# teddyjfpender/tstwo

Measured on AMD Instinct MI355X. Metric: M31 CFFT elems/sec at log_size=22 (per step: CFFT evaluate + Blake2s Merkle commit + root all-gather), higher is better.
Workload: dtype u32

## Files before the change

tstwo_amd/csrc/common.h:

```cpp
#pragma once
#include <hip/hip_runtime.h>
#include <stdint.h>
#include <stdio.h>
#include <initializer_list>
#include <string>

#include "../../include/tstwo_hip.h"
#include "host_field.h"
#include "m31.cuh"

namespace tstwo {

struct Context {
    bool ready = false;
    int device = -1;
    hipStream_t own_stream = nullptr;
    hipStream_t stream = nullptr;
    cpoint *gen_pow2 = nullptr;
    cpoint *gen_win = nullptr;
    u32 *flag = nullptr;
    u32 *flag_host = nullptr;
    u32 *scratch = nullptr;
    size_t scratch_bytes = 0;
    int n_cus = 256;
    u32 **coltab = nullptr;
    size_t coltab_cap = 0;
    void *pinned = nullptr;
    void *result_host = nullptr;
    void *result_dev = nullptr;
    void *up_ring = nullptr;
    hipEvent_t up_done[16] = {};
    bool up_busy[16] = {};
    int up_next = 0;
    u32 *seq_host = nullptr;
    u32 *seq_dev = nullptr;
    u32 seq_next = 0;
    hipStream_t copy_stream[2] = {nullptr, nullptr};
    hipEvent_t copy_after = nullptr;
    hipEvent_t copy_done[2] = {nullptr, nullptr};
    bool copy_pending[2] = {false, false};
    int copy_next = 0;
};
constexpr size_t kPinnedBytes = 64 * 1024;
constexpr size_t kResultBytes = 256 * 1024;
constexpr int kUpSlots = 16;
constexpr int kCopyStreams = 2;
constexpr size_t kUpSlotBytes = 16 * 1024;

struct Knobs {
    int cfft_rounds = 1;
    int cfft_maxwg = 0;
    int cfft_lds_pad = 0;
    int cfft_kb = 0, cfft_ka = 0;
    int cfft_logta = 0;
    bool cfft_trace = false, cfft_sync = false;
    int merkle_cap = 32;
    int fold_cap = 64;
};
#ifdef TSTWO_EXPERIMENTS
const Knobs &knobs();
#else
inline constexpr Knobs kShippedKnobs{};
inline constexpr const Knobs &knobs() { return kShippedKnobs; }
#endif

Context &ctx();
int set_error(int code, const char *msg);
int set_error(int code, const std::string &msg);
int hip_fail(hipError_t e, const char *what);
int require_ready();
int ensure_scratch(size_t bytes);
bool stream_is_capturing();
int wait_stream();
int read_and_clear_flag(u32 *value);
int small_d2h(void *host_dst, const void *dev_src, size_t bytes);
void *result_target(size_t bytes);
int result_wait(const void **host_view);
int small_h2d(void *dev_dst, const void *host_src, size_t bytes);

#define TSTWO_HIP(call)                                        \
    do {                                                       \
        hipError_t _e = (call);                                \
        if (_e != hipSuccess) return ::tstwo::hip_fail(_e, #call); \
    } while (0)

#define TSTWO_REQUIRE_READY()                      \
    do {                                           \
        int _rc = ::tstwo::require_ready();        \
        if (_rc) return _rc;                       \
    } while (0)

#define TSTWO_LAUNCH_CHECK() TSTWO_HIP(hipGetLastError())

static inline unsigned ceil_div(size_t a, size_t b) { return (unsigned)((a + b - 1) / b); }

constexpr int kMaxColsPerLaunch = 64;
struct ColPtrs { u32 *p[kMaxColsPerLaunch]; u32 *const *ext; };
#ifdef __HIPCC__
typedef u32 u32x4_t __attribute__((ext_vector_type(4)));
typedef u32 u32x2_t __attribute__((ext_vector_type(2)));
#define TSTWO_GLOBAL __attribute__((address_space(1)))
__device__ __forceinline__ void raise_flag(u32 *flag) { *(volatile TSTWO_GLOBAL u32 *)flag = 1u; }
template <bool NT, class V>
__device__ __forceinline__ V gload_as(const TSTWO_GLOBAL V *p) {
    if constexpr (NT) return __builtin_nontemporal_load(p);
    else return *p;
}
template <bool NT, class V>
__device__ __forceinline__ void gstore_as(TSTWO_GLOBAL V *p, V v) {
    if constexpr (NT) __builtin_nontemporal_store(v, p);
    else *p = v;
}
template <bool NT = false>
__device__ __forceinline__ uint4 gload4(const u32 *p) {
    const u32x4_t v = gload_as<NT>((const TSTWO_GLOBAL u32x4_t *)p);
    return make_uint4(v.x, v.y, v.z, v.w);
}
__device__ __forceinline__ uint2 gload2(const u32 *p) {
    const u32x2_t v = *(const TSTWO_GLOBAL u32x2_t *)p;
    return make_uint2(v.x, v.y);
}
template <bool NT = false>
__device__ __forceinline__ u32 gload1(const u32 *p) { return gload_as<NT>((const TSTWO_GLOBAL u32 *)p); }
template <bool NT = false>
__device__ __forceinline__ void gstore4(u32 *p, uint4 x) {
    u32x4_t v;
    v.x = x.x; v.y = x.y; v.z = x.z; v.w = x.w;
    gstore_as<NT>((TSTWO_GLOBAL u32x4_t *)p, v);
}
template <bool NT = false>
__device__ __forceinline__ void gstore1(u32 *p, u32 x) { gstore_as<NT>((TSTWO_GLOBAL u32 *)p, x); }
template <bool NT = false>
__device__ __forceinline__ uint4 gload4(const u32 *base, u32 word_off) {
    const u32x4_t v = gload_as<NT>((const TSTWO_GLOBAL u32x4_t *)((const TSTWO_GLOBAL char *)base + (word_off << 2)));
    return make_uint4(v.x, v.y, v.z, v.w);
}
__device__ __forceinline__ uint2 gload2(const u32 *base, u32 word_off) {
    const u32x2_t v = *(const TSTWO_GLOBAL u32x2_t *)((const TSTWO_GLOBAL char *)base + (word_off << 2));
    return make_uint2(v.x, v.y);
}
template <bool NT = false>
__device__ __forceinline__ u32 gload1(const u32 *base, u32 word_off) { return gload_as<NT>((const TSTWO_GLOBAL u32 *)((const TSTWO_GLOBAL char *)base + (word_off << 2))); }
template <bool NT = false>
__device__ __forceinline__ void gstore4(u32 *base, u32 word_off, uint4 x) {
    u32x4_t v;
    v.x = x.x; v.y = x.y; v.z = x.z; v.w = x.w;
    gstore_as<NT>((TSTWO_GLOBAL u32x4_t *)((TSTWO_GLOBAL char *)base + (word_off << 2)), v);
}
__device__ __forceinline__ void gstore2(u32 *base, u32 word_off, uint2 x) {
    u32x2_t v;
    v.x = x.x; v.y = x.y;
    *(TSTWO_GLOBAL u32x2_t *)((TSTWO_GLOBAL char *)base + (word_off << 2)) = v;
}
template <bool NT = false>
__device__ __forceinline__ void gstore1(u32 *base, u32 word_off, u32 x) { gstore_as<NT>((TSTWO_GLOBAL u32 *)((TSTWO_GLOBAL char *)base + (word_off << 2)), x); }
__device__ __forceinline__ u32 *colp(const ColPtrs &c, u32 i) {
    u32 *p;
    if (c.ext) {
        asm volatile("");
        p = c.ext[i];
    } else {
        p = c.p[i];
    }
    return p;
}
template <int KERNARG_OFF = 0>
__device__ __forceinline__ u32 *colp_u(const ColPtrs &c, u32 i) {
    typedef const unsigned long long __attribute__((address_space(4))) *k64;
    typedef const char __attribute__((address_space(4))) *kbytes;
    const k64 tab = c.ext ? (k64)(unsigned long long)c.ext : (k64)((kbytes)__builtin_amdgcn_kernarg_segment_ptr() + KERNARG_OFF);
    u32 *p = (u32 *)tab[(u32)__builtin_amdgcn_readfirstlane((int)i)];
    return p;
}
constexpr int kSecondTableOff = (int)sizeof(ColPtrs);
#endif
int merkle_commit_then_channel(const u32 *const *cols, const u32 *log_sizes, size_t n_cols, uint8_t *layers, u32 *chan, u32 *felt,
                               const u32 *const *fold_in, const u32 *inv_x, const u32 *alpha_dev);
int launch_fri_tail(u32 *const (*eval)[4], uint8_t *const *trees, u32 n_layers, u32 log0, const u32 *itw, u32 tw_log, u32 *chan, u32 *alphas,
                    const u32 *const *pre, const u32 *pre_alpha);
__attribute__((visibility("hidden"))) int download_roots(const uint8_t *const *layers, size_t n_trees, uint8_t *roots);
__attribute__((visibility("hidden"))) void air_native_shutdown();
int fill_col_table(ColPtrs &out, const u32 *const *cols, size_t n_cols, int slot);
constexpr int kMaxHashCols = 256;
struct HashColPtrs { const u32 *p[kMaxHashCols]; };
struct Soa4 { u32 *p[4]; };
struct CSoa4 { const u32 *p[4]; };

inline bool has_null(std::initializer_list<const void *> l) {
    for (const void *p : l) if (!p) return true;
    return false;
}
template <typename T>
inline bool table_has_null(T *const *t, size_t n) {
    if (!t) return n > 0;
    for (size_t i = 0; i < n; i++) if (!t[i]) return true;
    return false;
}
#define TSTWO_REQUIRE_PTRS(...) do { if (::tstwo::has_null({__VA_ARGS__})) return set_error(TSTWO_ERR_BAD_ARG, "null device pointer"); } while (0)
#define TSTWO_REQUIRE_TABLE(t, n) do { if (::tstwo::table_has_null((t), (n))) return set_error(TSTWO_ERR_BAD_ARG, "null device pointer in table"); } while (0)
inline bool aligned16(const void *p) { return ((uintptr_t)p & 15) == 0; }
inline qm31 to_q(const u32 a[4]) { return {a[0], a[1], a[2], a[3]}; }
inline qm31 to_q(host::Q a) { return {a.v[0], a.v[1], a.v[2], a.v[3]}; }
inline host::Q to_hq(const u32 a[4]) { host::Q q; for (int i = 0; i < 4; i++) q.v[i] = a[i]; return q; }

}
```

tstwo_amd/csrc/context.hip:

```cpp
#include "common.h"

#include <stdlib.h>
#include <string.h>

#include <chrono>
#include <map>
#include <mutex>
#include <unordered_map>
#include <vector>

namespace tstwo {

static Context g_ctx;
static thread_local std::string g_last_error;

Context &ctx() { return g_ctx; }

#ifdef TSTWO_EXPERIMENTS
static Knobs read_knobs() {
    Knobs k;
    auto num = [](const char *name, int dflt) { const char *e = getenv(name); return e && *e ? atoi(e) : dflt; };
    auto on = [](const char *name) { return getenv(name) != nullptr; };
    k.cfft_rounds = num("TSTWO_CFFT_ROUNDS", 1); if (k.cfft_rounds < 1) k.cfft_rounds = 1;
    k.cfft_maxwg = num("TSTWO_CFFT_MAXWG", 0); if (k.cfft_maxwg < 0) k.cfft_maxwg = 0;
    k.cfft_lds_pad = num("TSTWO_CFFT_LDS_PAD", 0);
    k.cfft_kb = num("TSTWO_CFFT_KB", 0); if (k.cfft_kb < 11 || k.cfft_kb > 15) k.cfft_kb = 0;
    k.cfft_ka = num("TSTWO_CFFT_KA", 0); if (k.cfft_ka < 1 || k.cfft_ka > 10) k.cfft_ka = 0;
    k.cfft_logta = num("TSTWO_CFFT_LOGTA", 0); if (k.cfft_logta < 12 || k.cfft_logta > 15) k.cfft_logta = 0;
    k.cfft_trace = on("TSTWO_CFFT_TRACE"); k.cfft_sync = on("TSTWO_CFFT_SYNC");
    k.merkle_cap = num("TSTWO_MERKLE_CAP", 32);
    k.fold_cap = num("TSTWO_FOLD_CAP", 64);
    return k;
}
const Knobs &knobs() {
    static const Knobs k = read_knobs();
    return k;
}
#endif

int set_error(int code, const char *msg) {
    g_last_error = msg ? msg : "";
    return code;
}
int set_error(int code, const std::string &msg) {
    g_last_error = msg;
    return code;
}
int hip_fail(hipError_t e, const char *what) {
    g_last_error = std::string("HIP error: ") + hipGetErrorString(e) + " in " + what;
    (void)hipGetLastError();
    return TSTWO_ERR_HIP;
}
int require_ready() {
    if (!g_ctx.ready) {
        int rc = tstwo_init(0);
        if (rc) return rc;
    }
    return TSTWO_OK;
}
bool stream_is_capturing() {
    hipStreamCaptureStatus st = hipStreamCaptureStatusNone;
    if (hipStreamIsCapturing(g_ctx.stream, &st) != hipSuccess) { (void)hipGetLastError(); return false; }
    return st != hipStreamCaptureStatusNone;
}
static std::vector<void *> g_scratch_retired;
int ensure_scratch(size_t bytes) {
    Context &c = g_ctx;
    if (c.scratch_bytes >= bytes) return TSTWO_OK;
    size_t want = bytes < (1u << 20) ? (1u << 20) : bytes;
    if (c.scratch) {
        if (stream_is_capturing())
            return set_error(TSTWO_ERR_BAD_ARG, "scratch growth during graph capture (run the sequence once eagerly first: the "
                                                "library's scratch block must already hold what the captured calls need)");
        if (want < 2 * c.scratch_bytes) want = 2 * c.scratch_bytes;
    }
    u32 *grown = nullptr;
    TSTWO_HIP(hipMalloc((void **)&grown, want));
    if (c.scratch) g_scratch_retired.push_back(c.scratch);
    c.scratch = grown;
    c.scratch_bytes = want;
    return TSTWO_OK;
}
__global__ void k_signal(u32 *seq, u32 value) { *(volatile TSTWO_GLOBAL u32 *)seq = value; }
int wait_stream() {
    Context &c = g_ctx;
    if (!c.seq_host) {
        TSTWO_HIP(hipStreamSynchronize(c.stream));
        return TSTWO_OK;
    }
    const u32 want = ++c.seq_next;
    hipLaunchKernelGGL(k_signal, dim3(1), dim3(1), 0, c.stream, c.seq_dev, want);
    if (hipGetLastError() != hipSuccess) {
        TSTWO_HIP(hipStreamSynchronize(c.stream));
        return TSTWO_OK;
    }
    const auto t0 = std::chrono::steady_clock::now();
    for (unsigned spins = 0;; spins++) {
        if (__atomic_load_n(c.seq_host, __ATOMIC_ACQUIRE) == want) return TSTWO_OK;
        if ((spins & 255u) == 255u && std::chrono::steady_clock::now() - t0 > std::chrono::microseconds(100)) break;
    }
    TSTWO_HIP(hipStreamSynchronize(c.stream));
    return TSTWO_OK;
}
int small_d2h(void *host_dst, const void *dev_src, size_t bytes) {
    Context &c = g_ctx;
    if (bytes == 0) return TSTWO_OK;
    if (!c.pinned || bytes > kPinnedBytes) {
        TSTWO_HIP(hipMemcpyAsync(host_dst, dev_src, bytes, hipMemcpyDeviceToHost, c.stream));
        TSTWO_HIP(hipStreamSynchronize(c.stream));
        return TSTWO_OK;
    }
    TSTWO_HIP(hipMemcpyAsync(c.pinned, dev_src, bytes, hipMemcpyDeviceToHost, c.stream));
    if (int rc = wait_stream()) return rc;
    memcpy(host_dst, c.pinned, bytes);
    return TSTWO_OK;
}
void *result_target(size_t bytes) {
    Context &c = g_ctx;
    return (c.result_dev && bytes <= kResultBytes) ? c.result_dev : nullptr;
}
int result_wait(const void **host_view) {
    Context &c = g_ctx;
    if (int rc = wait_stream()) return rc;
    *host_view = c.result_host;
    return TSTWO_OK;
}
static int refuse_if_capturing() {
    if (stream_is_capturing())
        return set_error(TSTWO_ERR_BAD_ARG, "host-array upload during graph capture (column tables beyond 64 pointers, gather "
                                            "requests and quotient constants cannot be recorded)");
    return TSTWO_OK;
}
int small_h2d(void *dev_dst, const void *host_src, size_t bytes) {
    Context &c = g_ctx;
    if (bytes == 0) return TSTWO_OK;
    if (int rc = refuse_if_capturing()) return rc;
    if (!c.up_ring || bytes > kUpSlotBytes) {
        TSTWO_HIP(hipMemcpyAsync(dev_dst, host_src, bytes, hipMemcpyHostToDevice, c.stream));
        TSTWO_HIP(hipStreamSynchronize(c.stream));
        return TSTWO_OK;
    }
    const int k = c.up_next;
    c.up_next = (k + 1) % kUpSlots;
    if (c.up_busy[k]) TSTWO_HIP(hipEventSynchronize(c.up_done[k]));
    unsigned char *slot = (unsigned char *)c.up_ring + (size_t)k * kUpSlotBytes;
    memcpy(slot, host_src, bytes);
    TSTWO_HIP(hipMemcpyAsync(dev_dst, slot, bytes, hipMemcpyHostToDevice, c.stream));
    TSTWO_HIP(hipEventRecord(c.up_done[k], c.stream));
    c.up_busy[k] = true;
    return TSTWO_OK;
}
static std::vector<const u32 *> g_coltab_last[2];
static u32 **g_coltab_last_base[2] = {nullptr, nullptr};
static void coltab_cache_reset() { for (int i = 0; i < 2; i++) { g_coltab_last[i].clear(); g_coltab_last_base[i] = nullptr; } }

int fill_col_table(ColPtrs &out, const u32 *const *cols, size_t n_cols, int slot) {
    Context &c = g_ctx;
    out.ext = nullptr;
    if (n_cols <= (size_t)kMaxColsPerLaunch) {
        for (size_t i = 0; i < (size_t)kMaxColsPerLaunch; i++) out.p[i] = const_cast<u32 *>(cols[i < n_cols ? i : 0]);
        return TSTWO_OK;
    }
    if (int rc = refuse_if_capturing()) return rc;
    if (c.coltab_cap < n_cols) {
        size_t cap = 1024;
        while (cap < n_cols) cap *= 2;
        if (c.coltab) {
            TSTWO_HIP(hipStreamSynchronize(c.stream));
            TSTWO_HIP(hipFree(c.coltab));
            c.coltab = nullptr;
            c.coltab_cap = 0;
            coltab_cache_reset();
        }
        TSTWO_HIP(hipMalloc((void **)&c.coltab, 2 * cap * sizeof(u32 *)));
        c.coltab_cap = cap;
    }
    u32 **dst = c.coltab + (size_t)(slot & 1) * c.coltab_cap;
    std::vector<const u32 *> &lc = g_coltab_last[slot & 1];
    u32 ***last_base = g_coltab_last_base;
    if (!(last_base[slot & 1] == dst && lc.size() == n_cols && memcmp(lc.data(), cols, n_cols * sizeof(u32 *)) == 0)) {
        int rc = small_h2d(dst, cols, n_cols * sizeof(u32 *));
        if (rc) return rc;
        lc.assign(cols, cols + n_cols);
// ... 536 lines not shown
```

tstwo_amd/csrc/merkle.hip:

```cpp
#include <string.h>

#include <vector>

#include "blake2s.cuh"
#include "common.h"

using namespace tstwo;
using namespace tstwo::b2s;

namespace {

struct LayerParams {
    u32 total_words;
    u32 w_begin;
    u32 w_end;
    u32 col_word0;
    u32 n_cols;
    u32 load_state;
    u32 is_final;
};

template <bool HAS_PREV>
__device__ __forceinline__ void load_block(u32 (&m)[16], const uint4 *__restrict__ prev, const HashColPtrs &cols,
                                           const LayerParams &lp, size_t node, u32 w) {
    if (HAS_PREV && w == 0) {
        const uint4 *c = prev + 4 * node;
        uint4 c0 = c[0], c1 = c[1], c2 = c[2], c3 = c[3];
        m[0] = c0.x; m[1] = c0.y; m[2] = c0.z; m[3] = c0.w; m[4] = c1.x; m[5] = c1.y; m[6] = c1.z; m[7] = c1.w;
        m[8] = c2.x; m[9] = c2.y; m[10] = c2.z; m[11] = c2.w; m[12] = c3.x; m[13] = c3.y; m[14] = c3.z; m[15] = c3.w;
    } else if (lp.n_cols == 0) {
#pragma unroll
        for (int k = 0; k < 16; k++) m[k] = 0u;
    } else {
        const u32 last = lp.n_cols - 1u;
#pragma unroll
        for (int k = 0; k < 16; k++) {
            const u32 ci = w + (u32)k - lp.col_word0;
            const u32 v = cols.p[min(ci, last)][node];
            m[k] = (ci <= last) ? v : 0u;
        }
    }
}

template <bool HAS_PREV>
__global__ void __launch_bounds__(256) k_merkle_layer(const uint4 *__restrict__ prev, HashColPtrs cols, uint4 *__restrict__ out,
                                                     size_t n_nodes, LayerParams lp) {
    const size_t stride = (size_t)gridDim.x * blockDim.x;
    const size_t node0 = (size_t)blockIdx.x * blockDim.x + threadIdx.x;
    const u32 W = lp.total_words;
    const u32 w_stop = lp.w_end < W ? lp.w_end : W;
    const u32 nb = w_stop > lp.w_begin ? (w_stop - lp.w_begin + 15u) / 16u : 1u;
    const u32 rows = (u32)((n_nodes + stride - 1) / stride);
    const u32 total = rows * nb;
    const size_t last_node = n_nodes - 1;

    u32 ma[16], mb[16], h[8];
    u32 j = 0, blk = 0;
    load_block<HAS_PREV>(ma, prev, cols, lp, min(node0, last_node), lp.w_begin);

#define MERKLE_STEP(CUR, NXT)                                                                                         \
    {                                                                                                                 \
        const size_t node = node0 + (size_t)j * stride;                                                               \
        const size_t nc = min(node, last_node);                                                                       \
        const u32 wc = lp.w_begin + 16u * blk;                                                                        \
        if (blk == 0) {                                                                                               \
            if (lp.load_state) {                                                                                      \
                uint4 a = out[2 * nc], b = out[2 * nc + 1];                                                           \
                h[0] = a.x; h[1] = a.y; h[2] = a.z; h[3] = a.w; h[4] = b.x; h[5] = b.y; h[6] = b.z; h[7] = b.w;       \
            } else {                                                                                                  \
                h[0] = IV0 ^ 0x01010020u; h[1] = IV1; h[2] = IV2; h[3] = IV3; h[4] = IV4; h[5] = IV5; h[6] = IV6; h[7] = IV7; \
            }                                                                                                         \
        }                                                                                                             \
        u32 jn = j, bn = blk + 1;                                                                                     \
        if (bn == nb) { bn = 0; jn = j + 1; }                                                                         \
        if (it + 1 < total)                                                                                           \
            load_block<HAS_PREV>(NXT, prev, cols, lp, min(node0 + (size_t)jn * stride, last_node), lp.w_begin + 16u * bn); \
        const u32 bytes_end = (wc + 16 < W ? wc + 16 : W) * 4u;                                                       \
        b2s_compress(h, CUR, bytes_end, lp.is_final && (wc + 16 >= W));                                               \
        if (blk + 1 == nb && node < n_nodes) {                                                                        \
            out[2 * node] = make_uint4(h[0], h[1], h[2], h[3]);                                                       \
            out[2 * node + 1] = make_uint4(h[4], h[5], h[6], h[7]);                                                   \
        }                                                                                                             \
        j = jn; blk = bn;                                                                                             \
    }

    for (u32 it = 0; it < total; it += 2) {
        MERKLE_STEP(ma, mb)
        if (it + 1 < total) {
            const u32 it_save = it;
            it = it_save + 1;
            MERKLE_STEP(mb, ma)
            it = it_save;
        }
    }
#undef MERKLE_STEP
}

constexpr int kMaxTrees = 8;
struct TreeSet { uint4 *t[kMaxTrees]; };
template <int NBLK>
__global__ void __launch_bounds__(256) k_merkle_leaf_static(HashColPtrs cols, TreeSet outs, size_t n_nodes) {
    uint4 *__restrict__ out = outs.t[blockIdx.y];
    const u32 col0 = blockIdx.y * (16 * NBLK);
    const size_t stride = (size_t)gridDim.x * blockDim.x;
    const size_t node0 = (size_t)blockIdx.x * blockDim.x + threadIdx.x;
    const u32 rows = (u32)((n_nodes + stride - 1) / stride);
    const size_t last_node = n_nodes - 1;
    u32 cur[16], nxt[16];
    auto word = [&](int k, u32 byte_off) -> u32 { return *(const TSTWO_GLOBAL u32 *)((const TSTWO_GLOBAL char *)cols.p[col0 + k] + byte_off); };
    {
        const u32 oc = (u32)min(node0, last_node) * 4u;
#pragma unroll
        for (int k = 0; k < 16; k++) cur[k] = word(k, oc);
    }
    u32 hp[8] = {0, 0, 0, 0, 0, 0, 0, 0};
    size_t pnode = n_nodes;
    for (u32 j = 0; j < rows; j++) {
        const size_t node = node0 + (size_t)j * stride;
        const size_t nn = min(node + stride, last_node);
        const size_t nc = min(node, last_node);
        u32 h[8] = {IV0 ^ 0x01010020u, IV1, IV2, IV3, IV4, IV5, IV6, IV7};
#pragma unroll
        for (int b = 0; b < NBLK; b++) {
            const int bn = (b + 1) % NBLK;
            const u32 src = (u32)((b + 1 < NBLK) ? nc : nn) * 4u;
#pragma unroll
            for (int k = 0; k < 16; k++) nxt[k] = word(16 * bn + k, src);
            if (b == 0 && pnode < n_nodes) {
                out[2 * pnode] = make_uint4(hp[0], hp[1], hp[2], hp[3]);
                out[2 * pnode + 1] = make_uint4(hp[4], hp[5], hp[6], hp[7]);
            }
            b2s_compress(h, cur, 64u * (b + 1), b == NBLK - 1);
#pragma unroll
            for (int k = 0; k < 16; k++) cur[k] = nxt[k];
        }
#pragma unroll
        for (int k = 0; k < 8; k++) hp[k] = h[k];
        pnode = node;
    }
    if (pnode < n_nodes) {
        out[2 * pnode] = make_uint4(hp[0], hp[1], hp[2], hp[3]);
        out[2 * pnode + 1] = make_uint4(hp[4], hp[5], hp[6], hp[7]);
    }
}

struct FoldSpec { const u32 *in[4]; const u32 *inv_x; const u32 *alpha; };
struct FoldRow { uint2 a, b, c, d; u32 t; };
__device__ __forceinline__ FoldRow fold_row_load(const FoldSpec &fs, size_t i) {
    return {gload2(fs.in[0] + 2 * i), gload2(fs.in[1] + 2 * i), gload2(fs.in[2] + 2 * i), gload2(fs.in[3] + 2 * i), gload1(fs.inv_x + i)};
}
__device__ __forceinline__ qm31 fold_row(const FoldRow &r, qm31 alpha) {
    const qm31 f0 = {m31_add(r.a.x, r.a.y), m31_add(r.b.x, r.b.y), m31_add(r.c.x, r.c.y), m31_add(r.d.x, r.d.y)};
    const qm31 f1 = qm31_mul_m31({m31_sub(r.a.x, r.a.y), m31_sub(r.b.x, r.b.y), m31_sub(r.c.x, r.c.y), m31_sub(r.d.x, r.d.y)}, r.t);
    return qm31_add(f0, qm31_mul(alpha, f1));
}

template <bool FOLD>
__global__ void __launch_bounds__(256) k_merkle_leaf4(u32 *__restrict__ c0, u32 *__restrict__ c1, u32 *__restrict__ c2, u32 *__restrict__ c3,
                                                     uint4 *__restrict__ out, size_t n_nodes, FoldSpec fs) {
    const size_t stride = (size_t)gridDim.x * blockDim.x;
    const size_t node0 = (size_t)blockIdx.x * blockDim.x + threadIdx.x;
    const u32 rows = (u32)((n_nodes + stride - 1) / stride);
    const size_t last_node = n_nodes - 1;
    auto word = [&](const u32 *col, u32 byte_off) -> u32 { return *(const TSTWO_GLOBAL u32 *)((const TSTWO_GLOBAL char *)col + byte_off); };
    const u32 o0 = (u32)min(node0, last_node) * 4u;
    u32 a = 0, b = 0, c = 0, d = 0;
    FoldRow fr = {};
    qm31 alpha = {0, 0, 0, 0};
    if (FOLD) {
        alpha = {fs.alpha[0], fs.alpha[1], fs.alpha[2], fs.alpha[3]};
        fr = fold_row_load(fs, min(node0, last_node));
    } else {
        a = word(c0, o0); b = word(c1, o0); c = word(c2, o0); d = word(c3, o0);
    }
    u32 hp[8] = {0, 0, 0, 0, 0, 0, 0, 0};
    size_t pnode = n_nodes;
    for (u32 j = 0; j < rows; j++) {
        const size_t node = node0 + (size_t)j * stride;
        const size_t nn = min(node + stride, last_node);
        const u32 on = (u32)nn * 4u;
        u32 na = 0, nb = 0, ncc = 0, nd = 0;
        FoldRow nfr = {};
        if (FOLD) {
            nfr = fold_row_load(fs, nn);
        } else {
            na = word(c0, on); nb = word(c1, on); ncc = word(c2, on); nd = word(c3, on);
        }
        if (pnode < n_nodes) {
            out[2 * pnode] = make_uint4(hp[0], hp[1], hp[2], hp[3]);
            out[2 * pnode + 1] = make_uint4(hp[4], hp[5], hp[6], hp[7]);
        }
        if (FOLD) {
            const qm31 r = fold_row(fr, alpha);
            a = r.a; b = r.b; c = r.c; d = r.d;
            if (node < n_nodes) { gstore1(c0 + node, a); gstore1(c1 + node, b); gstore1(c2 + node, c); gstore1(c3 + node, d); }
        }
        u32 h[8] = {IV0 ^ 0x01010020u, IV1, IV2, IV3, IV4, IV5, IV6, IV7};
        const u32 m[16] = {a, b, c, d, 0, 0, 0, 0, 0, 0, 0, 0, 0, 0, 0, 0};
        b2s_compress(h, m, 16u, true);
#pragma unroll
        for (int k = 0; k < 8; k++) hp[k] = h[k];
        pnode = node;
        if (FOLD) fr = nfr;
        else { a = na; b = nb; c = ncc; d = nd; }
    }
    if (pnode < n_nodes) {
        out[2 * pnode] = make_uint4(hp[0], hp[1], hp[2], hp[3]);
        out[2 * pnode + 1] = make_uint4(hp[4], hp[5], hp[6], hp[7]);
    }
}

__device__ __forceinline__ void merkle_inner_body(const uint4 *__restrict__ prev, uint4 *__restrict__ out, size_t n_nodes) {
    const size_t stride = (size_t)gridDim.x * blockDim.x;
    const size_t node0 = (size_t)blockIdx.x * blockDim.x + threadIdx.x;
    const u32 rows = (u32)((n_nodes + stride - 1) / stride);
    const size_t last_node = n_nodes - 1;
    uint4 c[4], cn[4];
    {
        const uint4 *p = prev + 4 * min(node0, last_node);
        c[0] = p[0]; c[1] = p[1]; c[2] = p[2]; c[3] = p[3];
    }
    u32 hp[8] = {0, 0, 0, 0, 0, 0, 0, 0};
    size_t pnode = n_nodes;
    for (u32 j = 0; j < rows; j++) {
        const size_t node = node0 + (size_t)j * stride;
        const uint4 *pn = prev + 4 * min(node + stride, last_node);
        cn[0] = pn[0]; cn[1] = pn[1]; cn[2] = pn[2]; cn[3] = pn[3];
        if (pnode < n_nodes) {
            out[2 * pnode] = make_uint4(hp[0], hp[1], hp[2], hp[3]);
            out[2 * pnode + 1] = make_uint4(hp[4], hp[5], hp[6], hp[7]);
        }
        u32 h[8] = {IV0 ^ 0x01010020u, IV1, IV2, IV3, IV4, IV5, IV6, IV7};
        const u32 m[16] = {c[0].x, c[0].y, c[0].z, c[0].w, c[1].x, c[1].y, c[1].z, c[1].w,
                           c[2].x, c[2].y, c[2].z, c[2].w, c[3].x, c[3].y, c[3].z, c[3].w};
        b2s_compress(h, m, 64u, true);
#pragma unroll
        for (int k = 0; k < 8; k++) hp[k] = h[k];
        pnode = node;
        c[0] = cn[0]; c[1] = cn[1]; c[2] = cn[2]; c[3] = cn[3];
    }
    if (pnode < n_nodes) {
        out[2 * pnode] = make_uint4(hp[0], hp[1], hp[2], hp[3]);
        out[2 * pnode + 1] = make_uint4(hp[4], hp[5], hp[6], hp[7]);
    }
}

__global__ void __launch_bounds__(256) k_merkle_inner(const uint4 *__restrict__ prev, uint4 *__restrict__ out, size_t n_nodes) {
    merkle_inner_body(prev, out, n_nodes);
}
__global__ void __launch_bounds__(256) k_merkle_inner_set(TreeSet ts, u32 log_out) {
    uint4 *layers = ts.t[blockIdx.y];
    merkle_inner_body(layers + 2 * (((size_t)1 << (log_out + 1)) - 1), layers + 2 * (((size_t)1 << log_out) - 1), (size_t)1 << log_out);
}

__device__ __forceinline__ u32 xslot(u32 chunk) { return chunk + (chunk >> 3); }
__global__ void __launch_bounds__(256) k_merkle_subtree2c(TreeSet ts, u32 log_child) {
    __shared__ uint4 xch[4][288];
    uint4 *__restrict__ layers = ts.t[blockIdx.y];
    const u32 lane = threadIdx.x & 63u;
    uint4 *x = xch[threadIdx.x >> 6];
    const size_t top0 = (size_t)blockIdx.x * 256u + (threadIdx.x & ~63u);
    const u32 *cbase = (const u32 *)(layers + 2 * ((((size_t)1 << log_child) - 1) + 4 * top0));
    uint4 in[8];
#pragma unroll
    for (int k = 0; k < 8; k++) in[k] = gload4(cbase, 4u * (64u * k + lane));
    Digest ch[4];
#pragma unroll
    for (int h = 0; h < 2; h++) {
#pragma unroll
        for (int k = 0; k < 4; k++) x[xslot(64u * k + lane)] = in[4 * h + k];
        asm volatile("" ::: "memory");
        if ((lane >> 5) == (u32)h) {
            const uint4 *mine = x + 9u * (lane & 31u);
#pragma unroll
            for (int j = 0; j < 4; j++) {
                const uint4 a = mine[2 * j], b = mine[2 * j + 1];
                ch[j] = {{a.x, a.y, a.z, a.w, b.x, b.y, b.z, b.w}};
            }
        }
        asm volatile("" ::: "memory");
    }
    const Digest l = hash_pair(ch[0], ch[1]);
    const Digest r = hash_pair(ch[2], ch[3]);
    const Digest top = hash_pair(l, r);
    {
        uint4 *mine = x + xslot(4u * lane);
        mine[0] = make_uint4(l.w[0], l.w[1], l.w[2], l.w[3]); mine[1] = make_uint4(l.w[4], l.w[5], l.w[6], l.w[7]);
        mine[2] = make_uint4(r.w[0], r.w[1], r.w[2], r.w[3]); mine[3] = make_uint4(r.w[4], r.w[5], r.w[6], r.w[7]);
    }
    asm volatile("" ::: "memory");
    uint4 o[4];
#pragma unroll
    for (int k = 0; k < 4; k++) o[k] = x[xslot(64u * k + lane)];
    asm volatile("" ::: "memory");
    {
        uint4 *mine = x + xslot(2u * lane);
        mine[0] = make_uint4(top.w[0], top.w[1], top.w[2], top.w[3]); mine[1] = make_uint4(top.w[4], top.w[5], top.w[6], top.w[7]);
    }
// ... 114 lines not shown
        if (parents_log >= 9 && remaining >= 9 && remaining <= 16) {
            hipLaunchKernelGGL(k_merkle_upq<1024>, dim3(1u << (parents_log - 8), n_trees), dim3(1024), 0, c.stream, ts, log_child, 9u, none);
            log_child -= 9;
        } else if (parents_log <= 6) {
            hipLaunchKernelGGL(k_merkle_upq<256>, dim3(1, n_trees), dim3(256), 0, c.stream, ts, log_child, remaining, root_hook);
            log_child -= remaining;
        } else if (parents_log <= 8) {
            hipLaunchKernelGGL(k_merkle_upq<1024>, dim3(1, n_trees), dim3(1024), 0, c.stream, ts, log_child, remaining, root_hook);
            log_child -= remaining;
        } else {
            u32 levels = remaining < 7 ? remaining : 7;
            hipLaunchKernelGGL(k_merkle_upq<256>, dim3(1u << (parents_log - 6), n_trees), dim3(256), 0, c.stream, ts, log_child, levels, none);
            log_child -= levels;
        }
    }
    TSTWO_LAUNCH_CHECK();
    return TSTWO_OK;
}

__global__ void __launch_bounds__(64) k_channel_mix_draw(u32 *__restrict__ chan, const u32 *__restrict__ root, u32 *__restrict__ felt,
                                                        u32 do_mix, u32 do_draw) {
    u32 d[8], f[4] = {0, 0, 0, 0};
#pragma unroll
    for (int k = 0; k < 8; k++) d[k] = chan[k];
    u32 n_chal = chan[8], n_sent = chan[9];
    chan_mix_draw(d, n_chal, n_sent, root, do_mix != 0, do_draw != 0, f);
    if (do_draw && threadIdx.x < 4) {
        u32 v = f[0];
        v = threadIdx.x == 1 ? f[1] : v;
        v = threadIdx.x == 2 ? f[2] : v;
        v = threadIdx.x == 3 ? f[3] : v;
        felt[threadIdx.x] = v;
    }
    if (threadIdx.x == 0) {
#pragma unroll
        for (int k = 0; k < 8; k++) chan[k] = d[k];
        chan[8] = n_chal;
        chan[9] = n_sent;
    }
}

struct FriTail {
    u32 *eval[11][4];
    uint4 *tree[10];
    u32 n_layers, log0;
    const u32 *pre[4];
    const u32 *pre_alpha;
};
__global__ void __launch_bounds__(1024) k_fri_tail(FriTail ft, const u32 *__restrict__ itw, u32 tw_log, u32 *__restrict__ chan,
                                                  u32 *__restrict__ alphas) {
    constexpr u32 Q = 256;
    __shared__ __attribute__((aligned(16))) u32 sh[Q * 16];
    __shared__ __attribute__((aligned(16))) u32 evl[4][512];
    __shared__ u32 alpha_sh[4];
    const u32 t = threadIdx.x;
    u32 d[8], n_chal = 0, n_sent = 0;
    if (t < 64) {
#pragma unroll
        for (int k = 0; k < 8; k++) d[k] = chan[k];
        n_chal = chan[8]; n_sent = chan[9];
    }
    u32 row[4] = {0u, 0u, 0u, 0u};
    if (t < (1u << ft.log0)) {
        if (ft.pre_alpha) {
            const qm31 alpha = *reinterpret_cast<const qm31 *>(ft.pre_alpha);
            const u32 tw0 = gload1(itw + ((size_t)1 << tw_log) - ((size_t)2 << ft.log0) + t);
            const uint2 a = gload2(ft.pre[0] + 2 * t), b = gload2(ft.pre[1] + 2 * t), c = gload2(ft.pre[2] + 2 * t), e = gload2(ft.pre[3] + 2 * t);
            const qm31 f0 = {m31_add(a.x, a.y), m31_add(b.x, b.y), m31_add(c.x, c.y), m31_add(e.x, e.y)};
            const qm31 f1 = qm31_mul_m31({m31_sub(a.x, a.y), m31_sub(b.x, b.y), m31_sub(c.x, c.y), m31_sub(e.x, e.y)}, tw0);
            const qm31 r0 = qm31_add(f0, qm31_mul(alpha, f1));
            row[0] = r0.a; row[1] = r0.b; row[2] = r0.c; row[3] = r0.d;
#pragma unroll
            for (int c2 = 0; c2 < 4; c2++) { gstore1(ft.eval[0][c2] + t, row[c2]); evl[c2][t] = row[c2]; }
        } else {
#pragma unroll
            for (int c = 0; c < 4; c++) { row[c] = gload1(ft.eval[0][c] + t); evl[c][t] = row[c]; }
        }
    }
    for (u32 i = 0; i < ft.n_layers; i++) {
        const u32 lg = ft.log0 - i;
        uint4 *layers = ft.tree[i];
        const u32 active = 1u << (lg - 1);
        const u32 tw = t < active ? gload1(itw + ((size_t)1 << tw_log) - ((size_t)1 << lg) + t) : 0u;
        if (t < 2 * active) leaf4_to_lds(layers, lg, t, sh, t, row[0], row[1], row[2], row[3]);
        lds_only_barrier();
        upq_levels<1024>(layers, sh, lg, lg, active, 0u);
        if (t < 64) {
            u32 f[4];
            chan_mix_draw(d, n_chal, n_sent, sh, true, true, f);
            if (t < 4) {
                const u32 v = t == 0 ? f[0] : t == 1 ? f[1] : t == 2 ? f[2] : f[3];
                alpha_sh[t] = v;
                alphas[4 * i + t] = v;
            }
        }
        lds_only_barrier();
        qm31 r = {0u, 0u, 0u, 0u};
        if (t < active) {
            const qm31 alpha = {alpha_sh[0], alpha_sh[1], alpha_sh[2], alpha_sh[3]};
            const uint2 a = *reinterpret_cast<const uint2 *>(&evl[0][2 * t]), b = *reinterpret_cast<const uint2 *>(&evl[1][2 * t]),
                        c = *reinterpret_cast<const uint2 *>(&evl[2][2 * t]), e = *reinterpret_cast<const uint2 *>(&evl[3][2 * t]);
            const qm31 f0 = {m31_add(a.x, a.y), m31_add(b.x, b.y), m31_add(c.x, c.y), m31_add(e.x, e.y)};
            const qm31 f1 = qm31_mul_m31({m31_sub(a.x, a.y), m31_sub(b.x, b.y), m31_sub(c.x, c.y), m31_sub(e.x, e.y)}, tw);
            r = qm31_add(f0, qm31_mul(alpha, f1));
            gstore1(ft.eval[i + 1][0] + t, r.a); gstore1(ft.eval[i + 1][1] + t, r.b);
            gstore1(ft.eval[i + 1][2] + t, r.c); gstore1(ft.eval[i + 1][3] + t, r.d);
        }
        lds_only_barrier();
        if (t < active) { evl[0][t] = r.a; evl[1][t] = r.b; evl[2][t] = r.c; evl[3][t] = r.d; }
        row[0] = r.a; row[1] = r.b; row[2] = r.c; row[3] = r.d;
        lds_only_barrier();
    }
    if (t == 0) {
#pragma unroll
        for (int k = 0; k < 8; k++) chan[k] = d[k];
        chan[8] = n_chal;
        chan[9] = n_sent;
    }
}

struct GrindDigest { u32 w[8]; };
__global__ void __launch_bounds__(256) k_grind(GrindDigest d, u32 pow_bits, unsigned long long base, unsigned long long count,
                                              unsigned long long *__restrict__ best) {
    const unsigned long long i = (unsigned long long)blockIdx.x * blockDim.x + threadIdx.x;
    if (i >= count) return;
    const unsigned long long nonce = base + i;
    u32 m[16] = {d.w[0], d.w[1], d.w[2], d.w[3], d.w[4], d.w[5], d.w[6], d.w[7], (u32)nonce, (u32)(nonce >> 32), 0, 0, 0, 0, 0, 0};
    u32 h[8] = {IV0 ^ 0x01010020u, IV1, IV2, IV3, IV4, IV5, IV6, IV7};
    b2s_compress(h, m, 40u, true);
    u32 tz = 0;
    if (h[0]) tz = __ffs(h[0]) - 1;
    else if (h[1]) tz = 32 + __ffs(h[1]) - 1;
    else if (h[2]) tz = 64 + __ffs(h[2]) - 1;
    else if (h[3]) tz = 96 + __ffs(h[3]) - 1;
    else tz = 128;
    if (tz >= pow_bits) atomicMin(best, nonce);
}

unsigned layer_blocks(size_t n_nodes, unsigned n_trees) {
    const unsigned blocks = ceil_div(n_nodes, 256);
    const unsigned cap = (unsigned)ctx().n_cus * (unsigned)knobs().merkle_cap / n_trees;
    return blocks <= cap ? blocks : cap ? cap : 1;
}

int launch_leaf_static(const HashColPtrs &hp, size_t cols_per_tree, const TreeSet &leaf, unsigned n_trees, u32 log_size) {
    const size_t n_nodes = (size_t)1 << log_size;
    const dim3 grid(layer_blocks(n_nodes, n_trees), n_trees);
    hipStream_t stream = ctx().stream;
    switch (cols_per_tree / 16) {
        case 1: hipLaunchKernelGGL(k_merkle_leaf_static<1>, grid, dim3(256), 0, stream, hp, leaf, n_nodes); break;
        case 2: hipLaunchKernelGGL(k_merkle_leaf_static<2>, grid, dim3(256), 0, stream, hp, leaf, n_nodes); break;
        case 3: hipLaunchKernelGGL(k_merkle_leaf_static<3>, grid, dim3(256), 0, stream, hp, leaf, n_nodes); break;
        default: hipLaunchKernelGGL(k_merkle_leaf_static<4>, grid, dim3(256), 0, stream, hp, leaf, n_nodes); break;
    }
    TSTWO_LAUNCH_CHECK();
    return TSTWO_OK;
}

int commit_column_free(const TreeSet &ts, unsigned n_trees, u32 log_child, u32 log_stop, ChanHook *hook) {
    hipStream_t stream = ctx().stream;
    for (; log_child >= log_stop + 2 && log_child - 2 >= (u32)kUpLog; log_child -= 2) {
        const size_t tops = (size_t)1 << (log_child - 2);
        hipLaunchKernelGGL(k_merkle_subtree2c, dim3((unsigned)(tops / 256), n_trees), dim3(256), 0, stream, ts, log_child);
    }
    if (log_child > log_stop && log_child - 1 >= (u32)kUpLog) {
        log_child -= 1;
        hipLaunchKernelGGL(k_merkle_inner_set, dim3(layer_blocks((size_t)1 << log_child, n_trees), n_trees), dim3(256), 0, stream, ts, log_child);
    }
    TSTWO_LAUNCH_CHECK();
    return commit_upper_levels(ts, n_trees, log_child, log_stop, hook);
}

int commit_layer(u32 log_size, const uint8_t *prev, const u32 *const *cols, size_t n_cols, uint8_t *out, const FoldSpec *fold) {
    Context &c = ctx();
    if (log_size > 31) return set_error(TSTWO_ERR_BAD_ARG, "merkle: log size out of range");
    if (!out) return set_error(TSTWO_ERR_BAD_ARG, "merkle: null output layer");
    if (!aligned16(out) || !aligned16(prev)) return set_error(TSTWO_ERR_BAD_ARG, "merkle: layers must be 16-byte aligned");
    if (fold && (prev || log_size > 30 || n_cols != 4)) return set_error(TSTWO_ERR_HIP, "fri commit: the fold was not carried by the leaf launch");
    const size_t n_nodes = (size_t)1 << log_size;
    const u32 child_words = prev ? 16u : 0u;
    const u32 W = child_words + (u32)n_cols;
    const unsigned blocks = layer_blocks(n_nodes, 1);
    if (!prev && log_size <= 30 && (n_cols == 16 || n_cols == 32 || n_cols == 48 || n_cols == 64)) {
        HashColPtrs hp;
        for (size_t k = 0; k < n_cols; k++) hp.p[k] = cols[k];
        TreeSet one = {};
        one.t[0] = (uint4 *)out;
        return launch_leaf_static(hp, n_cols, one, 1, log_size);
    }
    if (!prev && log_size <= 30 && n_cols == 4) {
        u32 *w0 = const_cast<u32 *>(cols[0]), *w1 = const_cast<u32 *>(cols[1]), *w2 = const_cast<u32 *>(cols[2]), *w3 = const_cast<u32 *>(cols[3]);
        if (fold)
            hipLaunchKernelGGL(k_merkle_leaf4<true>, dim3(blocks), dim3(256), 0, c.stream, w0, w1, w2, w3, (uint4 *)out, n_nodes, *fold);
        else
            hipLaunchKernelGGL(k_merkle_leaf4<false>, dim3(blocks), dim3(256), 0, c.stream, w0, w1, w2, w3, (uint4 *)out, n_nodes, FoldSpec{});
        TSTWO_LAUNCH_CHECK();
        return TSTWO_OK;
    }
    if (prev && n_cols == 0) {
        hipLaunchKernelGGL(k_merkle_inner, dim3(blocks), dim3(256), 0, c.stream, (const uint4 *)prev, (uint4 *)out, n_nodes);
        TSTWO_LAUNCH_CHECK();
        return TSTWO_OK;
    }
    size_t col_base = 0;
    bool first = true;
    do {
        size_t take = n_cols - col_base;
        if (take > (size_t)kMaxHashCols) take = kMaxHashCols;
        bool final_launch = (col_base + take == n_cols);
        if (!final_launch) {
            size_t end_word = child_words + col_base + take;
            take -= end_word % 16;
        }
        HashColPtrs hp;
        for (size_t k = 0; k < take; k++) hp.p[k] = cols[col_base + k];
        LayerParams lp;
        lp.total_words = W;
        lp.w_begin = first ? 0u : (u32)(child_words + col_base);
        lp.w_end = final_launch ? (W > 0 ? W : 1u) + 16u : (u32)(child_words + col_base + take);
        lp.col_word0 = (u32)(child_words + col_base);
        lp.n_cols = (u32)take;
        lp.load_state = first ? 0u : 1u;
        lp.is_final = final_launch ? 1u : 0u;
        if (prev)
            hipLaunchKernelGGL(k_merkle_layer<true>, dim3(blocks), dim3(256), 0, c.stream, (const uint4 *)prev, hp, (uint4 *)out, n_nodes, lp);
        else
            hipLaunchKernelGGL(k_merkle_layer<false>, dim3(blocks), dim3(256), 0, c.stream, (const uint4 *)nullptr, hp, (uint4 *)out, n_nodes, lp);
        col_base += take;
        first = false;
    } while (col_base < n_cols);
    TSTWO_LAUNCH_CHECK();
    return TSTWO_OK;
}

int commit_tree(const u32 *const *cols, const u32 *log_sizes, size_t n_cols, uint8_t *layers, uint8_t root[32], const FoldSpec *fold,
                ChanHook *hook) {
    TSTWO_REQUIRE_READY();
    if (!layers) return set_error(TSTWO_ERR_BAD_ARG, "merkle: null layers buffer");
    if (n_cols && !log_sizes) return set_error(TSTWO_ERR_BAD_ARG, "merkle: null log size table");
    TSTWO_REQUIRE_TABLE(cols, n_cols);
    u32 max_log = 0;
    for (size_t i = 0; i < n_cols; i++) {
        if (log_sizes[i] > 31) return set_error(TSTWO_ERR_BAD_ARG, "merkle: log size out of range");
        if (log_sizes[i] > max_log) max_log = log_sizes[i];
    }
    const auto has_cols = [&](u32 lg) {
        for (size_t i = 0; i < n_cols; i++)
            if (log_sizes[i] == lg) return true;
        return false;
    };
    TreeSet one = {};
    one.t[0] = (uint4 *)layers;
    if (n_cols == 4 && max_log >= 1 && (int)max_log <= kUpLog && log_sizes[0] == max_log && log_sizes[1] == max_log && log_sizes[2] == max_log &&
        log_sizes[3] == max_log) {
        u32 *w0 = const_cast<u32 *>(cols[0]), *w1 = const_cast<u32 *>(cols[1]), *w2 = const_cast<u32 *>(cols[2]), *w3 = const_cast<u32 *>(cols[3]);
        const FoldSpec fs = fold ? *fold : FoldSpec{};
        const bool whole = max_log <= 9;
        const u32 levels = whole ? max_log : 7u;
        const ChanHook hk = whole && hook ? *hook : ChanHook{nullptr, nullptr};
        const auto kernel = whole ? (fold ? k_merkle_leaf4_upq<1024, true> : k_merkle_leaf4_upq<1024, false>)
                                  : (fold ? k_merkle_leaf4_upq<256, true> : k_merkle_leaf4_upq<256, false>);
        hipLaunchKernelGGL(kernel, dim3(1u << (max_log - levels)), dim3(whole ? 1024 : 256), 0, ctx().stream, w0, w1, w2, w3, (uint4 *)layers,
                           max_log, levels, hk, fs);
        TSTWO_LAUNCH_CHECK();
        if (whole && hook) *hook = {nullptr, nullptr};
        int rc = whole ? TSTWO_OK : commit_upper_levels(one, 1, max_log - levels, 0, hook);
        if (rc) return rc;
        if (root) return small_d2h(root, layers, 32);
        return TSTWO_OK;
    }
    const u32 **lc = n_cols ? new const u32 *[n_cols] : nullptr;
    const uint8_t *prev = nullptr;
    int rc = TSTWO_OK;
    int lg = (int)max_log;
    while (lg >= 0 && rc == TSTWO_OK) {
        size_t k = 0;
        for (size_t i = 0; i < n_cols; i++)
            if (log_sizes[i] == (u32)lg) lc[k++] = cols[i];
        uint8_t *dst = layers + 32 * (((size_t)1 << lg) - 1);
        if (k == 0 && prev != nullptr) {
            int stop = lg;
            while (stop > 0 && !has_cols((u32)stop - 1)) stop--;
            rc = commit_column_free(one, 1, (u32)lg + 1, (u32)stop, hook);
            prev = layers + 32 * (((size_t)1 << stop) - 1);
            lg = stop - 1;
            continue;
        }
        rc = commit_layer((u32)lg, prev, lc, k, dst, prev ? nullptr : fold);
        prev = dst;
        lg--;
    }
    delete[] lc;
    if (rc) return rc;
    if (root) {
        int rc2 = small_d2h(root, layers, 32);
        if (rc2) return rc2;
    }
    return TSTWO_OK;
}
}

namespace tstwo {
int merkle_commit_then_channel(const u32 *const *cols, const u32 *log_sizes, size_t n_cols, uint8_t *layers, u32 *chan, u32 *felt,
                               const u32 *const *fold_in, const u32 *inv_x, const u32 *alpha_dev) {
    FoldSpec fs = {};
    if (fold_in) fs = {{fold_in[0], fold_in[1], fold_in[2], fold_in[3]}, inv_x, alpha_dev};
    ChanHook hook = {chan, felt};
    int rc = commit_tree(cols, log_sizes, n_cols, layers, nullptr, fold_in ? &fs : nullptr, &hook);
    if (rc) return rc;
    return hook.chan ? tstwo_channel_mix_root_draw_felt(chan, layers, felt) : TSTWO_OK;
}
int launch_fri_tail(u32 *const (*eval)[4], uint8_t *const *trees, u32 n_layers, u32 log0, const u32 *itw, u32 tw_log, u32 *chan, u32 *alphas,
                    const u32 *const *pre, const u32 *pre_alpha) {
    if (n_layers == 0 || n_layers > 10 || log0 < n_layers || log0 > 9 || log0 - n_layers + 1 < 1)
        return set_error(TSTWO_ERR_BAD_ARG, "fri tail: layer range out of bounds");
    FriTail ft = {};
    for (u32 i = 0; i <= n_layers; i++)
        for (int k = 0; k < 4; k++) ft.eval[i][k] = eval[i][k];
    for (u32 i = 0; i < n_layers; i++) ft.tree[i] = (uint4 *)trees[i];
    ft.n_layers = n_layers;
    ft.log0 = log0;
    if (pre && pre_alpha) {
        if (tw_log > 31 || log0 + 1 > tw_log) return set_error(TSTWO_ERR_TWIDDLES, "Not enough twiddles!");
        for (int k = 0; k < 4; k++) ft.pre[k] = pre[k];
        ft.pre_alpha = pre_alpha;
    }
    hipLaunchKernelGGL(k_fri_tail, dim3(1), dim3(1024), 0, ctx().stream, ft, itw, tw_log, chan, alphas);
    TSTWO_LAUNCH_CHECK();
    return TSTWO_OK;
}
}

extern "C" {

size_t tstwo_merkle_layers_bytes(u32 max_log) { return 32u * (((size_t)2 << max_log) - 1); }

int tstwo_grind_blake2s(const uint8_t digest[32], u32 pow_bits, uint64_t start_nonce, uint64_t *nonce_out) {
    TSTWO_REQUIRE_READY();
    if (!digest || !nonce_out) return set_error(TSTWO_ERR_BAD_ARG, "grind: null argument");
    if (pow_bits > 128) return set_error(TSTWO_ERR_BAD_ARG, "grind: pow_bits > 128");
    Context &c = ctx();
    int rc = ensure_scratch(64);
    if (rc) return rc;
    unsigned long long *best = (unsigned long long *)c.scratch;
    GrindDigest d;
    for (int i = 0; i < 8; i++)
        d.w[i] = (u32)digest[4 * i] | ((u32)digest[4 * i + 1] << 8) | ((u32)digest[4 * i + 2] << 16) | ((u32)digest[4 * i + 3] << 24);
    unsigned long long base = start_nonce;
    const unsigned long long none = ~0ull;
    for (;;) {
        unsigned long long batch = 1ull << 20;
        if (base - start_nonce >= (1ull << 22)) batch = 1ull << 26;
        if (none - base < batch) batch = none - base;
        if (batch == 0) return set_error(TSTWO_ERR_BAD_ARG, "grind: nonce space exhausted");
        TSTWO_HIP(hipMemsetAsync(best, 0xFF, sizeof(none), c.stream));
        hipLaunchKernelGGL(k_grind, dim3((unsigned)((batch + 255) / 256)), dim3(256), 0, c.stream, d, pow_bits, base, batch, best);
        TSTWO_LAUNCH_CHECK();
        unsigned long long found = none;
        { int rc2 = small_d2h(&found, best, sizeof(found)); if (rc2) return rc2; }
        if (found != none) { *nonce_out = found; return TSTWO_OK; }
        base += batch;
    }
}

int tstwo_channel_mix_root_draw_felt(u32 *chan, const uint8_t *root, u32 *felt) {
    TSTWO_REQUIRE_READY();
    TSTWO_REQUIRE_PTRS(chan);
    if ((((uintptr_t)root) & 3) || (((uintptr_t)felt) & 3)) return set_error(TSTWO_ERR_BAD_ARG, "channel: unaligned pointer");
    hipLaunchKernelGGL(k_channel_mix_draw, dim3(1), dim3(64), 0, ctx().stream, chan, (const u32 *)root, felt, root ? 1u : 0u, felt ? 1u : 0u);
    TSTWO_LAUNCH_CHECK();
    return TSTWO_OK;
}

int tstwo_merkle_commit_layer(u32 log_size, const uint8_t *prev, const u32 *const *cols, size_t n_cols, uint8_t *out) {
    TSTWO_REQUIRE_READY();
    if (n_cols && !cols) return set_error(TSTWO_ERR_BAD_ARG, "merkle: null column table");
    TSTWO_REQUIRE_TABLE(cols, n_cols);
    return commit_layer(log_size, prev, cols, n_cols, out, nullptr);
}

int tstwo_merkle_commit(const u32 *const *cols, const u32 *log_sizes, size_t n_cols, uint8_t *layers, uint8_t root[32]) {
    return commit_tree(cols, log_sizes, n_cols, layers, root, nullptr, nullptr);
}


int tstwo_merkle_commit_many(const tstwo_commit_request *reqs, size_t n_trees, uint8_t *roots) {
    TSTWO_REQUIRE_READY();
    if (n_trees && !reqs) return set_error(TSTWO_ERR_BAD_ARG, "merkle: null request table");
    bool uniform = n_trees >= 2 && n_trees <= (size_t)kMaxTrees;
    size_t n_cols = n_trees ? reqs[0].n_cols : 0;
    u32 lg = 0;
    for (size_t r = 0; r < n_trees && uniform; r++) {
        const tstwo_commit_request &q = reqs[r];
        if (!q.layers || !q.cols || !q.log_sizes) return set_error(TSTWO_ERR_BAD_ARG, "merkle: null argument");
        uniform = q.n_cols == n_cols && (n_cols == 16 || n_cols == 32 || n_cols == 48 || n_cols == 64) && n_cols * n_trees <= (size_t)kMaxHashCols &&
                  aligned16(q.layers);
        for (size_t k = 0; k < q.n_cols && uniform; k++) {
            if (!q.cols[k]) return set_error(TSTWO_ERR_BAD_ARG, "null device pointer in table");
            if (r == 0 && k == 0) lg = q.log_sizes[0];
            uniform = q.log_sizes[k] == lg;
        }
    }
    uniform = uniform && lg >= (u32)kUpLog + 1 && lg <= 30;
    if (!uniform) {
        for (size_t r = 0; r < n_trees; r++) {
            int rc = tstwo_merkle_commit(reqs[r].cols, reqs[r].log_sizes, reqs[r].n_cols, reqs[r].layers, nullptr);
            if (rc) return rc;
        }
    } else {
        HashColPtrs hp;
        TreeSet leaf = {}, ts = {};
        for (size_t r = 0; r < n_trees; r++) {
            for (size_t k = 0; k < n_cols; k++) hp.p[r * n_cols + k] = reqs[r].cols[k];
            ts.t[r] = (uint4 *)reqs[r].layers;
            leaf.t[r] = (uint4 *)(reqs[r].layers + 32 * (((size_t)1 << lg) - 1));
        }
        int rc = launch_leaf_static(hp, n_cols, leaf, (unsigned)n_trees, lg);
        if (rc == TSTWO_OK) rc = commit_column_free(ts, (unsigned)n_trees, lg, 0, nullptr);
        if (rc) return rc;
    }
    if (!roots) return TSTWO_OK;
    std::vector<const uint8_t *> trees(n_trees);
    for (size_t r = 0; r < n_trees; r++) trees[r] = reqs[r].layers;
    return download_roots(trees.data(), n_trees, roots);
}

}
```

Baseline: 178.3 billion.

## Fuse Merkle leaf hashing with first inner level via paired-row kernel

Adds a leaf kernel in which each thread hashes two adjacent rows, using 8-byte loads per column, and also computes their parent hash. This produces the leaf layer and the next layer in one launch. It aims to remove one full pass over the leaf layer and one kernel launch for large uniform trees. It also software-pipelines column loads across compression blocks. In exchange, register pressure rises with double buffers for two rows, and the path is used only for aligned columns at or above a log-size threshold (default 19).

```diff
diff --git a/tstwo_amd/csrc/common.h b/tstwo_amd/csrc/common.h
--- a/tstwo_amd/csrc/common.h
+++ b/tstwo_amd/csrc/common.h
@@ -55,6 +55,7 @@
     int cfft_logta = 0;
     bool cfft_trace = false, cfft_sync = false;
     int merkle_cap = 32;
+    int merkle_pair_log = 19;
     int fold_cap = 64;
 };
 #ifdef TSTWO_EXPERIMENTS
diff --git a/tstwo_amd/csrc/context.hip b/tstwo_amd/csrc/context.hip
--- a/tstwo_amd/csrc/context.hip
+++ b/tstwo_amd/csrc/context.hip
@@ -29,6 +29,7 @@
     k.cfft_logta = num("TSTWO_CFFT_LOGTA", 0); if (k.cfft_logta < 12 || k.cfft_logta > 15) k.cfft_logta = 0;
     k.cfft_trace = on("TSTWO_CFFT_TRACE"); k.cfft_sync = on("TSTWO_CFFT_SYNC");
     k.merkle_cap = num("TSTWO_MERKLE_CAP", 32);
+    k.merkle_pair_log = num("TSTWO_MERKLE_PAIR_LOG", 19); if (k.merkle_pair_log < 1) k.merkle_pair_log = 1;
     k.fold_cap = num("TSTWO_FOLD_CAP", 64);
     return k;
 }
diff --git a/tstwo_amd/csrc/merkle.hip b/tstwo_amd/csrc/merkle.hip
--- a/tstwo_amd/csrc/merkle.hip
+++ b/tstwo_amd/csrc/merkle.hip
@@ -1,5 +1,6 @@
 #include <string.h>
 
+#include <type_traits>
 #include <vector>
 
 #include "blake2s.cuh"
@@ -144,6 +145,75 @@
     }
 }
 
+#ifndef TSTWO_MERKLE_PAIR_NT
+#define TSTWO_MERKLE_PAIR_NT 0
+#endif
+constexpr bool kPairNT = TSTWO_MERKLE_PAIR_NT != 0;
+template <int NBLK, bool NT>
+__global__ void __launch_bounds__(256) k_merkle_leaf_pair(HashColPtrs cols, TreeSet outs, size_t n_pairs) {
+    uint4 *__restrict__ leaf = outs.t[blockIdx.y];
+    uint4 *__restrict__ up = outs.t[blockIdx.y] - 2 * n_pairs;
+    const u32 col0 = blockIdx.y * (16 * NBLK);
+    const u32 np = (u32)n_pairs, stride = gridDim.x * blockDim.x, pair0 = blockIdx.x * blockDim.x + threadIdx.x;
+    const u32 rows = (np + stride - 1) / stride;
+    const u32 last_pair = np - 1;
+    u32 ca[16], cb[16], na[16], nb[16];
+    auto words = [&](int k, u32 byte_off, u32 &a, u32 &b) {
+        const u32x2_t v = gload_as<NT>((const TSTWO_GLOBAL u32x2_t *)((const TSTWO_GLOBAL char *)cols.p[col0 + k] + byte_off));
+        a = v.x; b = v.y;
+    };
+    {
+        const u32 oc = min(pair0, last_pair) * 8u;
+#pragma unroll
+        for (int k = 0; k < 16; k++) words(k, oc, ca[k], cb[k]);
+    }
+    u32 hp[8] = {0, 0, 0, 0, 0, 0, 0, 0};
+    u32 ppair = np;
+    for (u32 j = 0; j < rows; j++) {
+        const u32 pair = pair0 + j * stride;
+        const u32 pn = min(pair + stride, last_pair);
+        const u32 pc = min(pair, last_pair);
+        Digest A = {{IV0 ^ 0x01010020u, IV1, IV2, IV3, IV4, IV5, IV6, IV7}}, B = A;
+        auto block = [&](auto bc) __attribute__((always_inline)) {
+            constexpr int b = decltype(bc)::value;
+            constexpr int bn = (b + 1) % NBLK;
+            u32 src = ((b + 1 < NBLK) ? pc : pn) * 8u;
+            asm volatile("" : "+v"(src));
+#pragma unroll
+            for (int k = 0; k < 8; k++) words(16 * bn + k, src, na[k], nb[k]);
+            if (b == 0 && ppair < np) {
+                up[2 * (size_t)ppair] = make_uint4(hp[0], hp[1], hp[2], hp[3]);
+                up[2 * (size_t)ppair + 1] = make_uint4(hp[4], hp[5], hp[6], hp[7]);
+            }
+            b2s_compress(A.w, ca, 64u * (b + 1), b == NBLK - 1);
+            asm volatile("" : "+v"(src));
+#pragma unroll
+            for (int k = 8; k < 16; k++) words(16 * bn + k, src, na[k], nb[k]);
+            b2s_compress(B.w, cb, 64u * (b + 1), b == NBLK - 1);
+#pragma unroll
+            for (int k = 0; k < 16; k++) { ca[k] = na[k]; cb[k] = nb[k]; }
+        };
+        block(std::integral_constant<int, 0>{});
+        if constexpr (NBLK > 1) block(std::integral_constant<int, 1>{});
+        if constexpr (NBLK > 2) block(std::integral_constant<int, 2>{});
+        if constexpr (NBLK > 3) block(std::integral_constant<int, 3>{});
+        if (pair < np) {
+            leaf[4 * (size_t)pair] = make_uint4(A.w[0], A.w[1], A.w[2], A.w[3]);
+            leaf[4 * (size_t)pair + 1] = make_uint4(A.w[4], A.w[5], A.w[6], A.w[7]);
+            leaf[4 * (size_t)pair + 2] = make_uint4(B.w[0], B.w[1], B.w[2], B.w[3]);
+            leaf[4 * (size_t)pair + 3] = make_uint4(B.w[4], B.w[5], B.w[6], B.w[7]);
+        }
+        const Digest top = hash_pair(A, B);
+#pragma unroll
+        for (int k = 0; k < 8; k++) hp[k] = top.w[k];
+        ppair = pair;
+    }
+    if (ppair < np) {
+        up[2 * (size_t)ppair] = make_uint4(hp[0], hp[1], hp[2], hp[3]);
+        up[2 * (size_t)ppair + 1] = make_uint4(hp[4], hp[5], hp[6], hp[7]);
+    }
+}
+
 struct FoldSpec { const u32 *in[4]; const u32 *inv_x; const u32 *alpha; };
 struct FoldRow { uint2 a, b, c, d; u32 t; };
 __device__ __forceinline__ FoldRow fold_row_load(const FoldSpec &fs, size_t i) {
@@ -564,6 +634,26 @@
         case 2: hipLaunchKernelGGL(k_merkle_leaf_static<2>, grid, dim3(256), 0, stream, hp, leaf, n_nodes); break;
         case 3: hipLaunchKernelGGL(k_merkle_leaf_static<3>, grid, dim3(256), 0, stream, hp, leaf, n_nodes); break;
         default: hipLaunchKernelGGL(k_merkle_leaf_static<4>, grid, dim3(256), 0, stream, hp, leaf, n_nodes); break;
+    }
+    TSTWO_LAUNCH_CHECK();
+    return TSTWO_OK;
+}
+
+bool leaf_takes_pair(u32 log_size, bool columns_below, const u32 *const *cols, size_t n_cols) {
+    if (!(log_size >= 1 && log_size <= 30 && (int)log_size >= knobs().merkle_pair_log && !columns_below)) return false;
+    for (size_t i = 0; i < n_cols; i++)
+        if ((uintptr_t)cols[i] & 7) return false;
+    return true;
+}
+int launch_leaf_pair(const HashColPtrs &hp, size_t cols_per_tree, const TreeSet &leaf, unsigned n_trees, u32 log_size) {
+    const size_t n_pairs = (size_t)1 << (log_size - 1);
+    const dim3 grid(layer_blocks(n_pairs, n_trees), n_trees);
+    hipStream_t stream = ctx().stream;
+    switch (cols_per_tree / 16) {
+        case 1: hipLaunchKernelGGL((k_merkle_leaf_pair<1, kPairNT>), grid, dim3(256), 0, stream, hp, leaf, n_pairs); break;
+        case 2: hipLaunchKernelGGL((k_merkle_leaf_pair<2, kPairNT>), grid, dim3(256), 0, stream, hp, leaf, n_pairs); break;
+        case 3: hipLaunchKernelGGL((k_merkle_leaf_pair<3, kPairNT>), grid, dim3(256), 0, stream, hp, leaf, n_pairs); break;
+        default: hipLaunchKernelGGL((k_merkle_leaf_pair<4, kPairNT>), grid, dim3(256), 0, stream, hp, leaf, n_pairs); break;
     }
     TSTWO_LAUNCH_CHECK();
     return TSTWO_OK;
@@ -696,6 +786,16 @@
             rc = commit_column_free(one, 1, (u32)lg + 1, (u32)stop, hook);
             prev = layers + 32 * (((size_t)1 << stop) - 1);
             lg = stop - 1;
+            continue;
+        }
+        if (!prev && !fold && (k == 16 || k == 32 || k == 48 || k == 64) && aligned16(dst) && leaf_takes_pair((u32)lg, has_cols((u32)lg - 1), lc, k)) {
+            HashColPtrs hp;
+            for (size_t i = 0; i < k; i++) hp.p[i] = lc[i];
+            TreeSet leaf = {};
+            leaf.t[0] = (uint4 *)dst;
+            rc = launch_leaf_pair(hp, k, leaf, 1, (u32)lg);
+            prev = layers + 32 * (((size_t)1 << (lg - 1)) - 1);
+            lg -= 2;
             continue;
         }
         rc = commit_layer((u32)lg, prev, lc, k, dst, prev ? nullptr : fold);
@@ -827,8 +927,9 @@
             ts.t[r] = (uint4 *)reqs[r].layers;
             leaf.t[r] = (uint4 *)(reqs[r].layers + 32 * (((size_t)1 << lg) - 1));
         }
-        int rc = launch_leaf_static(hp, n_cols, leaf, (unsigned)n_trees, lg);
-        if (rc == TSTWO_OK) rc = commit_column_free(ts, (unsigned)n_trees, lg, 0, nullptr);
+        const bool pair = leaf_takes_pair(lg, false, hp.p, n_cols * n_trees);
+        int rc = pair ? launch_leaf_pair(hp, n_cols, leaf, (unsigned)n_trees, lg) : launch_leaf_static(hp, n_cols, leaf, (unsigned)n_trees, lg);
+        if (rc == TSTWO_OK) rc = commit_column_free(ts, (unsigned)n_trees, pair ? lg - 1 : lg, 0, nullptr);
         if (rc) return rc;
     }
     if (!roots) return TSTWO_OK;
```

New measurement: 180.3 billion, median of 6. 1.01x the previous value.
